# willSapgreen/stereo-vision

Measured on AMD Instinct MI355X. Metric: stereo pairs/sec (ELAS 1242x375, ROBOTICS, D1+D2+LR), higher is better.
Workload: dtype u8

## Files before the change

### include/svh.h

```cpp
#ifndef SVH_H
#define SVH_H

#include <stddef.h>
#include <stdint.h>

#ifdef __cplusplus
extern "C" {
#endif

#define SVH_OK                 0
#define SVH_ERR_FEW_SUPPORT    1
#define SVH_ERR_BAD_ARG       -1
#define SVH_ERR_HIP           -2
#define SVH_ERR_UNSUPPORTED   -3
#define SVH_ERR_NO_DEVICE     -4
#define SVH_ERR_BAD_DIMS      -7

typedef struct svh_elas_params {
    int32_t disp_min;
    int32_t disp_max;
    float   support_threshold;
    int32_t support_texture;
    int32_t candidate_stepsize;
    int32_t incon_window_size;
// ... 96 lines not shown
int32_t svh_elas_stream_push_device(svh_elas_stream* s, const uint8_t* dI1, const uint8_t* dI2,
                                    float* dD1, float* dD2, uint64_t* ticket);
int32_t svh_elas_stream_flush(svh_elas_stream* s);
int32_t svh_elas_stream_pop(svh_elas_stream* s, uint64_t* ticket, int32_t* status, int32_t timeout_ms);
int32_t svh_elas_stream_close(svh_elas_stream* s);
int32_t svh_elas_stream_push_device_n(svh_elas_stream* s, int32_t n, const uint8_t* dI1, const uint8_t* dI2,
                                      size_t in_stride, float* dD1, float* dD2, size_t out_stride,
                                      uint64_t* first_ticket);
int32_t svh_elas_stream_pop_n(svh_elas_stream* s, int32_t n, int32_t* status, int32_t* popped);
int32_t svh_elas_stream_push_n(svh_elas_stream* s, int32_t n, const uint8_t* const* I1, const uint8_t* const* I2,
                               float* const* D1, float* const* D2, uint64_t* first_ticket);

#define SVH_DISP_F32 0
#define SVH_DISP_U16 1
#define SVH_MAPS_BOTH 0
#define SVH_MAPS_LEFT 1
typedef struct { int32_t format; int32_t maps; } svh_elas_output;
int32_t svh_elas_process_out(svh_elas* e, const uint8_t* I1, const uint8_t* I2, void* D1, void* D2,
                             const int32_t* dims, const svh_elas_output* out);
int32_t svh_elas_process_batch_out(svh_elas* e, int32_t n, const uint8_t* const* I1, const uint8_t* const* I2,
                                   void* const* D1, void* const* D2, const int32_t* dims, int32_t* status,
                                   const svh_elas_output* out);
svh_elas_stream* svh_elas_stream_open_out(svh_elas* e, const int32_t* dims, int32_t depth, const svh_elas_output* out);
int32_t svh_elas_stream_push_out(svh_elas_stream* s, const uint8_t* I1, const uint8_t* I2, void* D1, void* D2,
                                 uint64_t* ticket);
int32_t svh_elas_stream_push_out_n(svh_elas_stream* s, int32_t n, const uint8_t* const* I1, const uint8_t* const* I2,
                                   void* const* D1, void* const* D2, uint64_t* first_ticket);
int32_t svh_disparity_pack_u16(const float* D, int32_t d_on_device, int64_t n, uint16_t* out, int32_t out_on_device);
int32_t svh_disparity_unpack_u16(const uint16_t* v, int64_t n, float* out);

int64_t svh_elas_trim(void);

int32_t svh_elas_set_lanes(int32_t lanes);
int32_t svh_elas_set_group(int32_t pairs);

int32_t svh_elas_set_stage(int32_t where);
void svh_elas_stage_stats(int64_t* device_groups, int64_t* handed_back);
void svh_elas_sizing_stats(int64_t* out4);
void svh_elas_get_settings(int32_t out[4]);

enum svh_elas_stage {
    SVH_ELAS_DESC1 = 0,
    SVH_ELAS_DESC2,
    SVH_ELAS_DCAN_RAW,
    SVH_ELAS_SUPPORT,
    SVH_ELAS_TRI1,
    SVH_ELAS_TRI2,
    SVH_ELAS_PLANES1,
    SVH_ELAS_PLANES2,
    SVH_ELAS_GRID1,
    SVH_ELAS_GRID2,
    SVH_ELAS_D1_RAW,
    SVH_ELAS_D2_RAW,
    SVH_ELAS_D1_LR,
    SVH_ELAS_D2_LR,
    SVH_ELAS_D1_SEG,
    SVH_ELAS_D2_SEG,
    SVH_ELAS_D1_GAP,
    SVH_ELAS_D2_GAP,
    SVH_ELAS_STAGE_COUNT
};
int32_t svh_elas_set_taps(svh_elas* e, int32_t enable);
int32_t svh_elas_get_stage(svh_elas* e, int32_t stage, void* buf, size_t cap, size_t* size);

int32_t svh_elas_last_timing(svh_elas* e, const char** names, float* ms, int32_t cap);

// ... 183 lines not shown
```

### stereo-vision_amd/csrc/elas_engine.cpp

```cpp
#include <hip/hip_runtime.h>
#include <stdio.h>
#include <string.h>

#include <atomic>
#include <chrono>
#include <condition_variable>
#include <deque>
#include <functional>
#include <algorithm>
#include <map>
#include <memory>
#include <mutex>
#include <string>
#include <thread>
#include <vector>

#include "hip_guard.h"
#include "svh_internal.h"

namespace svh {

static thread_local int t_device = 0;

#define HIP_TRY(kind, expr) SVH_HIP_TRY(nullptr, kind, expr)
#define LANE_GROW(buf, bytes) SVH_HIP_GROW(nullptr, buf, bytes)

struct KernelStat {
    double total_ms = 0;
    int64_t launches = 0;
};
static std::mutex g_prof_mu;
static std::map<std::string, KernelStat> g_prof;
static std::atomic<int> g_prof_on{0};
static char g_prof_only[64] = "";

struct EventProfiler : Profiler {
    hipStream_t stream = nullptr;
    std::vector<hipEvent_t> ev;
    std::vector<const char*> names;
    size_t used = 0;
    bool skipping = false;
    void begin(const char* kernel) override {
        skipping = g_prof_only[0] && strcmp(kernel, g_prof_only) != 0;
        if (skipping) return;
        if (ev.size() < 2 * (used + 1)) {
            hipEvent_t a, b;
            if (hipEventCreate(&a) != hipSuccess || hipEventCreate(&b) != hipSuccess) return;
            ev.push_back(a);
            ev.push_back(b);
            names.push_back(kernel);
        }
        names[used] = kernel;
        (void)hipEventRecord(ev[2 * used], stream);
    }
    void end() override {
        if (skipping || ev.size() < 2 * (used + 1)) return;
        (void)hipEventRecord(ev[2 * used + 1], stream);
        used++;
    }
    void collect() {
        if (!used) return;
        std::lock_guard<std::mutex> lk(g_prof_mu);
        for (size_t i = 0; i < used; i++) {
            float ms = 0;
            if (hipEventElapsedTime(&ms, ev[2 * i], ev[2 * i + 1]) == hipSuccess) {
                KernelStat& k = g_prof[names[i]];
                k.total_ms += ms;
                k.launches++;
            }
        }
        used = 0;
    }
};

struct LaneBufs {
    HipBuf<uint8_t> img;
    HipBuf<uint8_t> desc;
    HipBuf<int16_t> dcan;
    HipBuf<int32_t> owner;
    HipBuf<uint8_t> prior_dev;
    HipBuf<TriRaster> raster;
    HipBuf<float> planes;
    HipBuf<uint32_t> seed, mask;
    HipBuf<uint16_t> lists;
    HipBuf<float> Draw;
    HipBuf<float> D;
    HipBuf<float> tmp;
    HipBuf<uint16_t> U;
    HipBuf<int32_t> labels, counts;
    HipBuf<int32_t> seg_nroots;
    HipBuf<uint8_t> stage_blob;
    PinnedBuf<int16_t> h_dcan;
    PinnedBuf<uint8_t> h_img, h_prior;
    PinnedBuf<StageCounts> h_counts;
};

struct Lane : LaneBufs {
    EventProfiler prof;
    int device = 0;
    hipStream_t stream = nullptr;
    hipEvent_t wait_ev = nullptr;
    hipStream_t copy_stream = nullptr;
    hipEvent_t match_ev = nullptr, copy_ev = nullptr;
    bool poll_wait = false;
    bool parallel_host = true;
    bool lone_group = true;
    int32_t W = 0, H = 0, disp_max = -1, step = 0, grid_size = 0, sub = -1, gcap = 0;
    Dims d{};
    bool desc_fly = false;
    int64_t owner_hi = 0;
    size_t prior_cap = 0;
    size_t ntri_max = 0;
    std::vector<HostPrior> hp;
    std::vector<int32_t> P;
    StageDev stg{};
    bool stage_ok = false;
    hipEvent_t stage_ev = nullptr;
    bool resident = false;
    bool force_host = false;
    float P_key[5] = {-1, -1, -1, -1, -1};
    static constexpr int kHist = 4;
    int32_t hist_sup[kHist] = {}, hist_tri[kHist] = {};
    int hist_n = 0, hist_at = 0;
    int32_t hist_g = 0;
    svh_elas_params hist_p{};
    PhaseBSize sized{};
    size_t o_P = 0, o_sup = 0, o_tri = 0;

    void release() {
        if (!stream) return;
        (void)hipSetDevice(device);
        static_cast<LaneBufs&>(*this) = LaneBufs();
        stage_ok = false; stg = StageDev{};
        P_key[0] = -1;
        hist_n = 0;
        W = H = 0;
    }

    void destroy() {
        if (!stream) return;
        (void)hipSetDevice(device);
        release();
        for (hipEvent_t* e : {&wait_ev, &match_ev, &copy_ev, &stage_ev})
            if (*e) {
                (void)hipEventDestroy(*e);
                *e = nullptr;
            }
        for (hipEvent_t e : prof.ev) (void)hipEventDestroy(e);
        prof.ev.clear();
        prof.names.clear();
        if (copy_stream) (void)hipStreamDestroy(copy_stream);
        (void)hipStreamDestroy(stream);
        copy_stream = stream = nullptr;
    }

    int ensure(const svh_elas_params& p, int32_t w, int32_t h, int32_t g) {
        if (!stream) {
            HIP_TRY(none, hipSetDevice(device));
            HIP_TRY(none, hipStreamCreateWithFlags(&stream, hipStreamNonBlocking));
        }
        const int32_t st = p.candidate_stepsize + (p.subsampling ? p.candidate_stepsize % 2 : 0);
        if (w == W && h == H && p.disp_max == disp_max && st == step && p.grid_size == grid_size &&
            p.subsampling == sub && g <= gcap)
            return SVH_OK;
        hipStream_t keep = stream;
        release();
        stream = keep;
        d = make_dims(p, w, h);
        const size_t N = (size_t)w * h, DN = (size_t)d.DW * d.DH, G2 = (size_t)2 * g;
        LANE_GROW(img, G2 * N);
        LANE_GROW(desc, G2 * N * 16);
        LANE_GROW(owner, G2 * N * sizeof(int32_t));
        HIP_TRY(copy, hipMemset(owner, 0, G2 * N * sizeof(int32_t)));
        owner_hi = svh::env("SVH_TEST_OWNER_HI") ? atoll(svh::env("SVH_TEST_OWNER_HI")) : 0;
        LANE_GROW(Draw, G2 * DN * sizeof(float));
        LANE_GROW(D, G2 * DN * sizeof(float));
        LANE_GROW(tmp, G2 * DN * sizeof(float));
        LANE_GROW(labels, G2 * DN * sizeof(int32_t));
        LANE_GROW(counts, G2 * DN * sizeof(int32_t));
        LANE_GROW(seg_nroots, G2 * (size_t)((d.DW + 63) / 64) * ((d.DH + 15) / 16) * sizeof(int32_t));
        const size_t nc = (size_t)d.Wc * d.Hc;
        LANE_GROW(dcan, g * nc * sizeof(int16_t));
        LANE_GROW(h_dcan, g * nc * sizeof(int16_t));
        LANE_GROW(h_img, G2 * N);
        const size_t nsup = nc + 6;
        ntri_max = 2 * nsup + 8;
        prior_cap = sizeof(GroupHdr) + (size_t)(p.disp_max + 1) * sizeof(int32_t) + 512 +
                    (size_t)g * (nsup * 3 + 2 * ntri_max * 3) * sizeof(int32_t);
        LANE_GROW(prior_dev, prior_cap);
        LANE_GROW(h_prior, prior_cap);
        LANE_GROW(raster, G2 * ntri_max * sizeof(TriRaster));
        LANE_GROW(planes, G2 * ntri_max * 6 * sizeof(float));
        const size_t gw_bytes = G2 * d.gw * d.gh * d.gwords * sizeof(uint32_t);
        LANE_GROW(seed, gw_bytes + G2 * sizeof(uint32_t));
        LANE_GROW(mask, gw_bytes);
        if (d.gwords <= 8) LANE_GROW(lists, G2 * d.gw * d.gh * 32 * sizeof(uint16_t));
        hp.resize(g);
        o_P = (sizeof(GroupHdr) + 63) & ~(size_t)63;
        o_sup = (o_P + (size_t)(p.disp_max + 1) * sizeof(int32_t) + 63) & ~(size_t)63;
        o_tri = (o_sup + (size_t)g * nsup * 3 * sizeof(int32_t) + 63) & ~(size_t)63;
// ... 30 lines not shown
            stg.rec_cap = (int32_t)rec;
            stage_ok = true;
        }
        HIP_TRY(wait, hipDeviceSynchronize());
        W = w; H = h; disp_max = p.disp_max; step = st; grid_size = p.grid_size; sub = p.subsampling;
        gcap = g;
        return SVH_OK;
    }
};

static std::atomic<int> g_wait_us{40};
static std::atomic<bool> g_hostprof{false};
static hipError_t lane_wait(Lane& L) {
    if (!L.poll_wait || g_wait_us <= 0) return hipStreamSynchronize(L.stream);
    if (!L.wait_ev) {
        hipError_t e = hipEventCreateWithFlags(&L.wait_ev, hipEventDisableTiming);
        if (e != hipSuccess) return e;
    }
    hipError_t e = hipEventRecord(L.wait_ev, L.stream);
    if (e != hipSuccess) return e;
    for (;;) {
        e = hipEventQuery(L.wait_ev);
        if (e != hipErrorNotReady) return e;
        std::this_thread::sleep_for(std::chrono::microseconds(g_wait_us.load(std::memory_order_relaxed)));
    }
}

struct Pool {
    std::mutex mu;
    std::condition_variable cv;
    std::vector<Lane*> lanes;
    std::vector<Lane*> free_list;
    int max_lanes = 4;
};

static std::mutex g_mu;

static std::map<int, Pool*>& g_pools = *new std::map<int, Pool*>();
static std::atomic<int> g_lanes{6};
static std::atomic<int> g_group{32};
static std::atomic<bool> g_group_set{false};
static std::atomic<int> g_stage_mode{-1};
static int stage_mode_from_env();
static void apply_config(const svh_config& c, int explicit_call) {
    if (explicit_call) {
        if (c.elas_workers > 0) svh_elas_set_lanes(c.elas_workers);
        if (c.elas_pairs_per_launch > 0) svh_elas_set_group(c.elas_pairs_per_launch);
        svh_elas_set_stage(c.elas_stage);
        if (c.wait_us >= 0) g_wait_us = c.wait_us;
    }
    if (const char* e = svh::env("SVH_WAIT_US")) g_wait_us = atoi(e);
    if (svh::env("SVH_STAGE")) g_stage_mode.store(stage_mode_from_env());
    g_hostprof = svh::env("SVH_HOST_PROF") != nullptr;
}
namespace { struct ConfigHook { ConfigHook() { svh::on_config(apply_config); } } g_config_hook; }
static int group_for(size_t N) {
    const int g = std::max(1, std::min(g_group.load(), kMaxGroup));
    if (g_group_set.load()) return g;
    size_t a = std::max<size_t>(1, std::min<size_t>(g, (size_t)32 * 1024 * 1024 / std::max<size_t>(N, 1)));
    size_t free_b = 0, total_b = 0;
    if (a > 1 && hipMemGetInfo(&free_b, &total_b) == hipSuccess && free_b > 0) {
        const size_t per_pair = 120 * std::max<size_t>(N, 1), sets = (size_t)2 * std::max(1, g_lanes.load());
        a = std::max<size_t>(1, std::min<size_t>(a, free_b / 2 / (per_pair * sets)));
    } else {
        (void)hipGetLastError();
    }
    return (int)a;
}

static Pool* pool_for(int device) {
    std::lock_guard<std::mutex> lk(g_mu);
    auto it = g_pools.find(device);
    if (it != g_pools.end()) return it->second;
    Pool* p = new Pool();
    g_pools[device] = p;
    return p;
}

static void acquire_lanes(int device, int count, Lane** out) {
    Pool* p = pool_for(device);
    std::unique_lock<std::mutex> lk(p->mu);
    p->max_lanes = 2 * g_lanes.load() + 2;
    for (;;) {
        const int can_make = p->max_lanes - (int)p->lanes.size();
        if ((int)p->free_list.size() + std::max(can_make, 0) >= count) {
            for (int i = 0; i < count; i++) {
                if (!p->free_list.empty()) {
                    out[i] = p->free_list.back();
                    p->free_list.pop_back();
                } else {
                    Lane* l = new Lane();
                    l->device = device;
                    p->lanes.push_back(l);
                    out[i] = l;
                }
            }
            return;
        }
        p->cv.wait(lk);
    }
}

static Lane* acquire_lane(int device) {
    Lane* l = nullptr;
    acquire_lanes(device, 1, &l);
    return l;
}

static void release_lane(Lane* l) {
    Pool* p = pool_for(l->device);
    {
        std::lock_guard<std::mutex> lk(p->mu);
        p->free_list.push_back(l);
    }
    p->cv.notify_all();
}

struct Taps {
    bool enabled = false;
    std::vector<uint8_t> data[SVH_ELAS_STAGE_COUNT];
};

}

struct svh_elas {
    svh_elas_params p;
    int device;
    svh::Taps taps;
// ... 75 lines not shown
};
static HostProfDump g_hp_dump;
#define HP_MARK(slot) do { if (g_hostprof) { uint64_t n_ = cpu_ns(); g_hp_ns[slot] += n_ - hp_t; hp_t = n_; } } while (0)

static int stage_mode_from_env() {
    const char* e = svh::env("SVH_STAGE");
    if (!e || !*e || !strcmp(e, "auto") || !strcmp(e, "-1")) return -1;
    if (!strcmp(e, "host") || !strcmp(e, "0")) return 0;
    if (!strcmp(e, "device") || !strcmp(e, "1")) return 1;
    fprintf(stderr, "svhip: SVH_STAGE=%s is not one of auto|-1, host|0, device|1: using auto\n", e);
    return -1;
}

static std::atomic<int64_t> g_stage_dev_groups{0}, g_stage_redo_groups{0};
static std::atomic<int64_t> g_sized_bound{0}, g_sized_hist{0}, g_short_tri{0}, g_short_sup{0};

static hipError_t event_wait(Lane& L, hipEvent_t ev) {
    if (!L.poll_wait || g_wait_us <= 0) return hipEventSynchronize(ev);
    for (;;) {
        hipError_t e = hipEventQuery(ev);
        if (e != hipErrorNotReady) return e;
        std::this_thread::sleep_for(std::chrono::microseconds(g_wait_us.load(std::memory_order_relaxed)));
    }
}

static int run_group_body(Lane& L, const svh_elas_params& p, const int32_t* dims, const GroupIO& io,
                          int32_t* status, Taps* taps, svh_elas* timing, int mode, int prefer_device);

static int run_group(Lane& L, const svh_elas_params& p, const int32_t* dims, const GroupIO& io,
                     int32_t* status, Taps* taps, svh_elas* timing, int mode = RG_ALL, int prefer_device = 0) {
    const int rc = run_group_body(L, p, dims, io, status, taps, timing, mode, prefer_device);
    if (rc == SVH_ERR_HIP) {
        const std::string keep = svh_last_error();
        if (L.stream) (void)hipStreamSynchronize(L.stream);
        if (L.copy_stream) (void)hipStreamSynchronize(L.copy_stream);
        (void)hipGetLastError();
        L.prof.used = 0;
        L.resident = false;
        L.force_host = false;
        L.P_key[0] = -1;
        fail(rc, keep);
    }
    return rc;
}

static int run_group_body(Lane& L, const svh_elas_params& p, const int32_t* dims, const GroupIO& io,
                          int32_t* status, Taps* taps, svh_elas* timing, int mode, int prefer_device) {
    const int32_t W = dims[0], H = dims[1], g = io.g;
    int rc = check_params(p, W, H);
    if (rc) return rc;
    if (g < 1 || g > kMaxGroup) return fail(SVH_ERR_BAD_ARG, "bad group size");
    HIP_TRY(none, hipSetDevice(L.device));
    rc = L.ensure(p, W, H, g);
    if (rc) return rc;
    if (g > 1) taps = nullptr;
    const Dims& d = L.d;
    const bool u16 = !io.out_device && io.format == SVH_DISP_U16;
    const int nmaps = !io.out_device && io.maps == SVH_MAPS_LEFT ? 1 : 2;
    const size_t DNu = ((size_t)d.DW * d.DH + 7) & ~(size_t)7;
    if (u16) LANE_GROW(L.U, (size_t)L.gcap * 2 * DNu * sizeof(uint16_t));
    hipStream_t s = L.stream;
    L.prof.stream = s;
    const LaunchCtx cx = {s, g_prof_on.load() ? &L.prof : nullptr, L.lone_group};
    const size_t N = (size_t)W * H, DN = (size_t)d.DW * d.DH;
    const size_t nc = (size_t)d.Wc * d.Hc;
    const bool tapping = taps && taps->enabled;
    double t0 = now_ms();
    uint64_t hp_t = g_hostprof ? cpu_ns() : 0;

    GroupHdr* hdr = reinterpret_cast<GroupHdr*>(L.h_prior.p);
    DevMaps out;
    if (io.out_device) {
        out.D[0] = io.dD[0]; out.D[1] = io.dD[1]; out.stride[0] = out.stride[1] = io.out_stride;
    } else {
        out.D[0] = L.D; out.D[1] = L.D + DN; out.stride[0] = out.stride[1] = 2 * DN;
    }
    bool early_d2 = false;
    int32_t plane_radius = 2;

    auto enqueue_phase_b = [&](size_t o_P, size_t o_sup, size_t o_tri, int32_t total_sup, int32_t total_tri,
                               int32_t tri_bound, const PhaseBSize& size) -> int {
        GroupDev G;
        G.hdr = reinterpret_cast<const GroupHdr*>(L.prior_dev.p);
        G.P = reinterpret_cast<const int32_t*>(L.prior_dev + o_P);
        G.support = reinterpret_cast<const int32_t*>(L.prior_dev + o_sup);
        G.tri = reinterpret_cast<const int32_t*>(L.prior_dev + o_tri);
        G.raster = L.raster;
        G.planes = L.planes;
        G.seed = L.seed;
        G.mask = L.mask;
        G.lists = L.lists;
        G.desc = L.desc;
        G.desc_fly = L.desc_fly ? 1 : 0;
        G.owner = L.owner;
        if (L.owner_hi + 1 + tri_bound >= INT32_MAX) {
            HIP_TRY(copy, hipMemsetAsync(L.owner, 0, (size_t)2 * L.gcap * N * sizeof(int32_t), s));
            L.owner_hi = 0;
        }
        G.owner_base = (int32_t)L.owner_hi;
        L.owner_hi += 1 + tri_bound;
        G.Draw = L.Draw;
        G.plane_radius = plane_radius;
        G.prior_absmax = 0;
        for (int32_t dd = 0; dd <= plane_radius && dd < (int32_t)L.P.size(); dd++)
            G.prior_absmax = std::max(G.prior_absmax, (int32_t)std::min<int64_t>(std::llabs((long long)L.P[dd]), INT32_MAX));
        launch_prior(cx, p, d, g, total_sup, total_tri, G, size);
        if (tapping) {
            const int32_t n1 = hdr->tri_end[0], n2 = hdr->tri_end[1] - hdr->tri_end[0];
            rc = tap_dev(L, taps, SVH_ELAS_PLANES1, L.planes.p, (size_t)6 * n1); if (rc) return rc;
            rc = tap_dev(L, taps, SVH_ELAS_PLANES2, L.planes.p + (size_t)6 * n1, (size_t)6 * n2); if (rc) return rc;
            const size_t words = (size_t)d.gw * d.gh * d.gwords;
            std::vector<uint32_t> m(2 * words);
            HIP_TRY(copy, hipMemcpyAsync(m.data(), L.mask, m.size() * sizeof(uint32_t), hipMemcpyDeviceToHost, s));
            HIP_TRY(wait, lane_wait(L));
            for (int k = 0; k < 2; k++) {
                std::vector<int32_t> gr;
                expand_grid(p, d, m.data() + k * words, gr);
                tap_host(taps, SVH_ELAS_GRID1 + k, gr.data(), gr.size());
            }
        }
        launch_owner(cx, p, d, g, total_tri, G, size);
        const bool tiles = !tapping && post_tiles_ok(p);
        const char* match_err = nullptr;
        const bool lr_done = launch_match(cx, p, d, g, G, &out, tapping, &match_err);
        if (match_err) return fail(SVH_ERR_HIP, std::string("launch_match: ") + match_err);
        early_d2 = !io.out_device && lr_done && !tapping && p.postprocess_only_left && !u16 && nmaps == 2;
        if (early_d2) {
            if (!L.copy_stream) {
                HIP_TRY(none, hipStreamCreateWithFlags(&L.copy_stream, hipStreamNonBlocking));
                HIP_TRY(none, hipEventCreateWithFlags(&L.match_ev, hipEventDisableTiming));
                HIP_TRY(none, hipEventCreateWithFlags(&L.copy_ev, hipEventDisableTiming));
            }
            HIP_TRY(none, hipEventRecord(L.match_ev, s));
        }
        if (tapping) {
            rc = tap_dev(L, taps, SVH_ELAS_D1_RAW, L.Draw.p, DN); if (rc) return rc;
            rc = tap_dev(L, taps, SVH_ELAS_D2_RAW, L.Draw.p + DN, DN); if (rc) return rc;
        }
        const PostScratch ps = {L.tmp, L.labels, L.counts, L.seg_nroots};
        const int nside = p.postprocess_only_left ? 1 : 2;
        if (!lr_done) launch_lr(cx, p, d, g, G, out);
        if (tapping) {
            rc = tap_dev(L, taps, SVH_ELAS_D1_LR, out.D[0], DN); if (rc) return rc;
            rc = tap_dev(L, taps, SVH_ELAS_D2_LR, out.D[1], DN); if (rc) return rc;
        }
        launch_segments(cx, p, d, g, nside, G, out, ps, !tiles);
        if (tapping) {
            rc = tap_dev(L, taps, SVH_ELAS_D1_SEG, out.D[0], DN); if (rc) return rc;
            rc = tap_dev(L, taps, SVH_ELAS_D2_SEG, out.D[1], DN); if (rc) return rc;
        }
        if (tiles) {
            launch_gap_mean_tiles(cx, p, d, g, nside, G, out, ps);
        } else {
            launch_gap(cx, p, d, g, nside, G, out, ps);
            if (tapping) {
                rc = tap_dev(L, taps, SVH_ELAS_D1_GAP, out.D[0], DN); if (rc) return rc;
                rc = tap_dev(L, taps, SVH_ELAS_D2_GAP, out.D[1], DN); if (rc) return rc;
            }
            if (p.filter_adaptive_mean) launch_adaptive_mean(cx, p, d, g, nside, G, out, ps);
            if (p.filter_median) launch_median(cx, d, g, nside, G, out, ps);
        }
        if (u16) {
            PackMap pm[2 * kMaxGroup];
            for (int32_t j = 0; j < g; j++)
                for (int k = 0; k < nmaps; k++)
                    pm[j * nmaps + k] = {(int64_t)(((size_t)2 * j + k) * DN), (int64_t)(((size_t)j * nmaps + k) * DNu), (int64_t)DN};
            launch_disp_pack(cx, L.D, L.U, pm, g * nmaps);
        }
        return SVH_OK;
    };

    static const bool strided = !(svh::env("SVH_D2H_STRIDED") && atoi(svh::env("SVH_D2H_STRIDED")) == 0);
    auto copy_map = [&](int k, hipStream_t cs, const int32_t* active) -> int {
        const size_t bytes = DN * (u16 ? sizeof(uint16_t) : sizeof(float));
        const size_t spitch = u16 ? (size_t)nmaps * DNu * sizeof(uint16_t) : 2 * bytes;
        for (int32_t j = 0; j < g;) {
            if (!active[j]) { j++; continue; }
            int32_t e = j + 1;
            while (strided && e < g && active[e] &&
                   reinterpret_cast<const char*>(io.hD[k][e]) == reinterpret_cast<const char*>(io.hD[k][e - 1]) + bytes)
                e++;
            const void* src = u16 ? (const void*)(L.U + ((size_t)j * nmaps + k) * DNu)
                                  : (const void*)(L.D + ((size_t)2 * j + k) * DN);
            if (e - j > 1)
                HIP_TRY(copy, hipMemcpy2DAsync(io.hD[k][j], bytes, src, spitch, bytes, (size_t)(e - j),
                                         hipMemcpyDeviceToHost, cs));
            else
                HIP_TRY(copy, hipMemcpyAsync(io.hD[k][j], src, bytes, hipMemcpyDeviceToHost, cs));
            g_d2h_map_bytes.fetch_add((int64_t)(bytes * (size_t)(e - j)), std::memory_order_relaxed);
            g_d2h_map_copies.fetch_add(1, std::memory_order_relaxed);
            j = e;
        }
        return SVH_OK;
    };
    auto copy_out = [&](const int32_t* active) -> int {
        if (io.out_device) return SVH_OK;
        if (early_d2) {
            HIP_TRY(none, hipStreamWaitEvent(L.copy_stream, L.match_ev, 0));
            rc = copy_map(1, L.copy_stream, active);
            if (rc) return rc;
// ... 100 lines not shown
                        uint8_t* dst = L.h_img + ((size_t)2 * j + k) * N;
                        const uint8_t* src = io.hI[k][j];
                        if (io.pitch == W) memcpy(dst, src, N);
                        else
                            for (int32_t v = 0; v < H; v++) memcpy(dst + (size_t)v * W, src + (size_t)v * io.pitch, W);
                    }
                HIP_TRY(copy, hipMemcpyAsync(L.img, L.h_img, (size_t)2 * g * N, hipMemcpyHostToDevice, s));
            }
            img.I[0] = L.img; img.I[1] = L.img + N;
            img.stride = 2 * N; img.pitch = W;
        }
        {
            std::vector<int32_t> Pt;
            int32_t pr = 2;
            prior_table(p, Pt, &pr);
            int32_t absmax = 0;
            for (int32_t dd = 0; dd <= pr && dd < (int32_t)Pt.size(); dd++)
                absmax = std::max(absmax, (int32_t)std::min<int64_t>(std::llabs((long long)Pt[dd]), INT32_MAX));
            static const int fly_env = svh::env("SVH_DESC_FLY") ? atoi(svh::env("SVH_DESC_FLY")) : 1;
            L.desc_fly = (!tapping || fly_env == 2) && descriptors_on_the_fly(p, d, absmax, pr, L.lists != nullptr);
        }
        if (tapping && L.desc_fly) {
            launch_descriptor(cx, img, g, W, H, p.subsampling, L.desc, false);
            int rc2 = tap_dev(L, taps, SVH_ELAS_DESC1, L.desc.p, N * 16); if (rc2) return rc2;
            rc2 = tap_dev(L, taps, SVH_ELAS_DESC2, L.desc.p + N * 16, N * 16); if (rc2) return rc2;
            HIP_TRY(wait, hipStreamSynchronize(s));
        }
        launch_descriptor(cx, img, g, W, H, p.subsampling, L.desc, L.desc_fly);
        launch_support(cx, p, d, g, L.desc, L.dcan, L.desc_fly);
        const int sm = g_stage_mode.load();
        L.resident = !L.force_host && L.stage_ok &&
                     (sm == 1 || (sm < 0 && prefer_device && stage_device_preferred(p, d, prefer_device > 1)));
        if (L.resident && prefer_device) L.poll_wait = true;
        if (!L.resident || tapping)
            HIP_TRY(copy, hipMemcpyAsync(L.h_dcan, L.dcan, g * nc * sizeof(int16_t), hipMemcpyDeviceToHost, s));
        if (L.resident) {
            prior_table(p, L.P, &plane_radius);
            const float key[5] = {p.beta, p.gamma, p.sigma, p.sradius, (float)p.disp_max};
            if (memcmp(key, L.P_key, sizeof(key)) != 0) {
                memcpy(L.h_prior + L.o_P, L.P.data(), L.P.size() * sizeof(int32_t));
                HIP_TRY(copy, hipMemcpyAsync(L.prior_dev + L.o_P, L.h_prior + L.o_P, L.P.size() * sizeof(int32_t),
                                       hipMemcpyHostToDevice, s));
                HIP_TRY(wait, hipStreamSynchronize(s));
                memcpy(L.P_key, key, sizeof(key));
            }
            if (tapping) {
                HIP_TRY(wait, hipStreamSynchronize(s));
                if (!L.desc_fly) {
                    rc = tap_dev(L, taps, SVH_ELAS_DESC1, L.desc.p, N * 16); if (rc) return rc;
                    rc = tap_dev(L, taps, SVH_ELAS_DESC2, L.desc.p + N * 16, N * 16); if (rc) return rc;
                }
                tap_host(taps, SVH_ELAS_DCAN_RAW, L.h_dcan.p, nc);
            }
            const bool blits = svh::env("SVH_STAGE_BLITS") && atoi(svh::env("SVH_STAGE_BLITS")) != 0;
            launch_stage_device(cx, p, d, g, L.stg, reinterpret_cast<GroupHdr*>(L.prior_dev.p),
                                reinterpret_cast<int32_t*>(L.prior_dev + L.o_sup),
                                reinterpret_cast<int32_t*>(L.prior_dev + L.o_tri),
                                blits ? nullptr : L.seed.p, seed_words_with_flags(d, g),
                                blits ? nullptr : L.h_counts.p);
            if (!L.stage_ev) HIP_TRY(none, hipEventCreateWithFlags(&L.stage_ev, hipEventDisableTiming));
            if (blits) HIP_TRY(copy, hipMemcpyAsync(L.h_counts, L.stg.counts, sizeof(StageCounts), hipMemcpyDeviceToHost, s));
            HIP_TRY(none, hipEventRecord(L.stage_ev, s));
            if (tapping) {
                HIP_TRY(copy, hipMemcpyAsync(hdr, L.prior_dev, sizeof(GroupHdr), hipMemcpyDeviceToHost, s));
                HIP_TRY(wait, hipStreamSynchronize(s));
                if (hdr->active[0]) {
                    rc = tap_dev(L, taps, SVH_ELAS_SUPPORT, reinterpret_cast<int32_t*>(L.prior_dev + L.o_sup),
                                 (size_t)3 * hdr->total_sup); if (rc) return rc;
                    rc = tap_dev(L, taps, SVH_ELAS_TRI1, reinterpret_cast<int32_t*>(L.prior_dev + L.o_tri),
                                 (size_t)3 * hdr->tri_end[0]); if (rc) return rc;
                    rc = tap_dev(L, taps, SVH_ELAS_TRI2,
                                 reinterpret_cast<int32_t*>(L.prior_dev + L.o_tri) + (size_t)3 * hdr->tri_end[0],
                                 (size_t)3 * (hdr->tri_end[1] - hdr->tri_end[0])); if (rc) return rc;
                }
            }
            L.sized = PhaseBSize{};
            if (!tapping || hdr->active[0]) {
                const int32_t tri_bound = 2 * g * 2 * L.stg.sup_cap;
                int32_t hint_sup = 0, hint_tri = 0;
                const bool use_hist = !(svh::env("SVH_PHASEB_HISTORY") && atoi(svh::env("SVH_PHASEB_HISTORY")) == 0);
                if (use_hist && L.hist_n && L.hist_g == g && memcmp(&L.hist_p, &p, sizeof(p)) == 0)
                    for (int k = 0; k < L.hist_n; k++) {
                        hint_sup = std::max(hint_sup, L.hist_sup[k]);
                        hint_tri = std::max(hint_tri, L.hist_tri[k]);
                    }
                L.sized = phase_b_size(d, g, -1, -1, hint_sup, hint_tri);
                L.sized.seed_cleared = !blits;
                rc = enqueue_phase_b(L.o_P, L.o_sup, L.o_tri, -1, -1, tri_bound, L.sized);
                if (rc) return rc;
            }
        }
        HP_MARK(HP_ENQ_A);
    }
    if (!(mode & RG_HOST_B)) return SVH_OK;
    double t1 = t0, t2 = t0;
    if (L.resident) {
        if (!io.out_device) {
            HIP_TRY(wait, event_wait(L, L.stage_ev));
            HP_MARK(HP_WAIT);
            int32_t active[kMaxGroup];
            for (int32_t j = 0; j < g; j++) active[j] = active_of(j);
            rc = copy_out(active);
            if (rc) return rc;
        }
        if (g_hostprof) g_hp_pairs += g;
        HP_MARK(HP_ENQ_B);
        t1 = t2 = now_ms();
    } else {
    const bool warm = L.parallel_host && g == 1;
    if (warm) helpers_warm(3, 1500);
    struct WarmOff {
        bool on;
        ~WarmOff() { if (on) helpers_warm(0, 0); }
    } warm_off{warm};
    HIP_TRY(wait, lane_wait(L));
    HIP_TRY(launch, hipGetLastError());
    L.prof.collect();
    HP_MARK(HP_WAIT);
    if (g_hostprof) g_hp_pairs += g;
    t1 = now_ms();
    if (tapping) {
        if (!L.desc_fly) {
// ... 888 lines not shown

void svh_test_d2h_map_bytes(int64_t out[2], int32_t reset) {
    if (out) {
        out[0] = svh::g_d2h_map_bytes.load();
        out[1] = svh::g_d2h_map_copies.load();
    }
    if (reset) {
        svh::g_d2h_map_bytes.store(0);
        svh::g_d2h_map_copies.store(0);
    }
}

void svh_elas_sizing_stats(int64_t* out4) {
    if (!out4) return;
    out4[0] = svh::g_sized_bound.load();
    out4[1] = svh::g_sized_hist.load();
    out4[2] = svh::g_short_tri.load();
    out4[3] = svh::g_short_sup.load();
}

void svh_elas_stage_stats(int64_t* device_groups, int64_t* handed_back) {
    if (device_groups) *device_groups = g_stage_dev_groups.load();
    if (handed_back) *handed_back = g_stage_redo_groups.load();
}

void svh_elas_get_settings(int32_t out[4]) {
    if (!out) return;
    out[0] = g_lanes.load();
    out[1] = g_group_set.load() ? g_group.load() : 0;
    out[2] = g_stage_mode.load();
    out[3] = g_wait_us;
}

int32_t svh_elas_set_group(int32_t pairs) {
    if (pairs < 1) pairs = 1;
    if (pairs > kMaxGroup) pairs = kMaxGroup;
    g_group.store(pairs);
    g_group_set.store(true);
    return pairs;
}

}
```

### stereo-vision_amd/svhip/__init__.py

```python
import ctypes as C
import os

import numpy as np

_HERE = os.path.dirname(os.path.abspath(__file__))
LIB_PATH = os.environ.get("SVH_LIB") or os.path.join(os.path.dirname(_HERE), "libsvhip.so")

OK, ERR_FEW_SUPPORT, ERR_BAD_ARG, ERR_HIP, ERR_UNSUPPORTED, ERR_NO_DEVICE = 0, 1, -1, -2, -3, -4
ERR_BAD_DIMS = -7
ROBOTICS, MIDDLEBURY = 0, 1


class ElasParams(C.Structure):
    _fields_ = [
        ("disp_min", C.c_int32), ("disp_max", C.c_int32),
        ("support_threshold", C.c_float), ("support_texture", C.c_int32),
        ("candidate_stepsize", C.c_int32), ("incon_window_size", C.c_int32),
        ("incon_threshold", C.c_int32), ("incon_min_support", C.c_int32),
        ("add_corners", C.c_int32), ("grid_size", C.c_int32),
        ("beta", C.c_float), ("gamma", C.c_float), ("sigma", C.c_float), ("sradius", C.c_float),
        ("match_texture", C.c_int32), ("lr_threshold", C.c_int32),
        ("speckle_sim_threshold", C.c_float), ("speckle_size", C.c_int32),
        ("ipol_gap_width", C.c_int32), ("filter_median", C.c_int32),
        ("filter_adaptive_mean", C.c_int32), ("postprocess_only_left", C.c_int32),
# ... 355 lines not shown

    def set_taps(self, enable=True):
        lib().svh_elas_set_taps(self._h, 1 if enable else 0)

    def stage(self, stage, dtype):
        n = C.c_size_t(0)
        lib().svh_elas_get_stage(self._h, stage, None, 0, C.byref(n))
        buf = np.empty(n.value, np.uint8)
        if n.value:
            rc = lib().svh_elas_get_stage(self._h, stage, buf.ctypes.data, n.value, C.byref(n))
            if rc < 0:
                raise SvhError(rc, last_error())
        return buf.view(dtype)

    def last_timing(self):
        names = (C.c_char_p * 16)()
        ms = (C.c_float * 16)()
        n = lib().svh_elas_last_timing(self._h, names, ms, 16)
        return [(names[i].decode(), ms[i]) for i in range(n)]


def set_lanes(n):
    return lib().svh_elas_set_lanes(n)


def set_group(n):
    return lib().svh_elas_set_group(n)


def set_stage(where):
    return lib().svh_elas_set_stage(where)


def trim():
    lib().svh_elas_trim.restype = C.c_int64
    return lib().svh_elas_trim()


def stage_stats():
    a, b = C.c_int64(0), C.c_int64(0)
    lib().svh_elas_stage_stats(C.byref(a), C.byref(b))
    return a.value, b.value


def device_count():
    return lib().svh_device_count()


def pack_u16(D):
    D = np.ascontiguousarray(D, np.float32)
    out = np.empty(D.shape, np.uint16)
    rc = lib().svh_disparity_pack_u16(D.ctypes.data, 0, D.size, out.ctypes.data, 0)
    if rc < 0:
        raise SvhError(rc, last_error())
    return out


def unpack_u16(v):
    v = np.ascontiguousarray(v, np.uint16)
    out = np.empty(v.shape, np.float32)
    rc = lib().svh_disparity_unpack_u16(v.ctypes.data, v.size, out.ctypes.data)
    if rc < 0:
        raise SvhError(rc, last_error())
    return out


# ... 454 lines not shown
```

Before: 35630.

## Split ELAS phases across priority-classed HIP streams per lane

Adds a queue plan that gives each lane up to three HIP streams with different priorities and routes phase A, the device staging phase and phase B (match, LR, postprocess) onto separate streams joined by events. Lanes of alternating parity can get low-priority streams, so concurrent lanes interleave better on the GPU's hardware queues. The auto plan picks by GPU_MAX_HW_QUEUES and the worker count, and falls back to a single stream when queues are plentiful or the budget is exceeded. This adds event synchronisation overhead, and the extra streams risk contending for the limited hardware queues.

```diff
diff --git a/include/svh.h b/include/svh.h
--- a/include/svh.h
+++ b/include/svh.h
@@ -152,6 +152,8 @@
 int64_t svh_elas_trim(void);
 
 int32_t svh_elas_set_lanes(int32_t lanes);
+int32_t svh_elas_set_queue_plan(int32_t plan);
+int32_t svh_elas_get_queue_plan(int32_t* plan, int32_t* streams_per_lane, int32_t* classes);
 int32_t svh_elas_set_group(int32_t pairs);
 
 int32_t svh_elas_set_stage(int32_t where);
diff --git a/stereo-vision_amd/csrc/elas_engine.cpp b/stereo-vision_amd/csrc/elas_engine.cpp
--- a/stereo-vision_amd/csrc/elas_engine.cpp
+++ b/stereo-vision_amd/csrc/elas_engine.cpp
@@ -16,6 +16,7 @@
 #include <vector>
 
 #include "hip_guard.h"
+#include "queue_plan.h"
 #include "svh_internal.h"
 
 namespace svh {
@@ -72,6 +73,20 @@
         used = 0;
     }
 };
+
+struct PhaseProfiler : Profiler {
+    EventProfiler* to;
+    hipStream_t stream;
+    PhaseProfiler(EventProfiler* t, hipStream_t s) : to(t), stream(s) {}
+    void begin(const char* kernel) override {
+        to->stream = stream;
+        to->begin(kernel);
+    }
+    void end() override { to->end(); }
+};
+
+static int queue_cap();
+static int worker_count();
 
 struct LaneBufs {
     HipBuf<uint8_t> img;
@@ -98,7 +113,15 @@
 struct Lane : LaneBufs {
     EventProfiler prof;
     int device = 0;
-    hipStream_t stream = nullptr;
+    hipStream_t stream = nullptr, stage_stream = nullptr, post_stream = nullptr;
+    hipStream_t cls_stream[QC_COUNT] = {nullptr, nullptr, nullptr};
+    int plan_req = QP_AUTO;
+    int parity = 0;
+    bool qp_known = false;
+    QueuePlan qp{};
+    int prio_least = 0, prio_greatest = 0;
+    bool split = false;
+    hipEvent_t a_ev = nullptr, b_ev = nullptr;
     hipEvent_t wait_ev = nullptr;
     hipStream_t copy_stream = nullptr;
     hipEvent_t match_ev = nullptr, copy_ev = nullptr;
@@ -138,10 +161,10 @@
     }
 
     void destroy() {
-        if (!stream) return;
+        if (!cls_stream[QC_NORMAL] && !cls_stream[QC_HIGH] && !cls_stream[QC_LOW]) return;
         (void)hipSetDevice(device);
         release();
-        for (hipEvent_t* e : {&wait_ev, &match_ev, &copy_ev, &stage_ev})
+        for (hipEvent_t* e : {&wait_ev, &match_ev, &copy_ev, &stage_ev, &a_ev, &b_ev})
             if (*e) {
                 (void)hipEventDestroy(*e);
                 *e = nullptr;
@@ -150,22 +173,48 @@
         prof.ev.clear();
         prof.names.clear();
         if (copy_stream) (void)hipStreamDestroy(copy_stream);
-        (void)hipStreamDestroy(stream);
-        copy_stream = stream = nullptr;
+        for (hipStream_t& cs : cls_stream)
+            if (cs) {
+                (void)hipStreamDestroy(cs);
+                cs = nullptr;
+            }
+        copy_stream = stream = stage_stream = post_stream = nullptr;
+    }
+
+    int bind_streams() {
+        if (!qp_known) {
+            HIP_TRY(none, hipSetDevice(device));
+            if (hipDeviceGetStreamPriorityRange(&prio_least, &prio_greatest) != hipSuccess) {
+                (void)hipGetLastError();
+                prio_least = prio_greatest = 0;
+            }
+            qp = make_queue_plan(prio_least, prio_greatest, queue_cap(), worker_count(), plan_req);
+            qp_known = true;
+        }
+        const QueueLane& ql = qp.lane[parity & 1];
+        for (int k = 0; k < ql.nstreams; k++) {
+            hipStream_t& cs = cls_stream[ql.cls[k]];
+            if (cs) continue;
+            HIP_TRY(none, hipSetDevice(device));
+            if (qp.plan == QP_ONE)
+                HIP_TRY(none, hipStreamCreateWithFlags(&cs, hipStreamNonBlocking));
+            else
+                HIP_TRY(none, hipStreamCreateWithPriority(&cs, hipStreamNonBlocking,
+                                                          queue_priority_of(ql.cls[k], prio_least, prio_greatest)));
+        }
+        stream = cls_stream[ql.cls[ql.phase_stream[QPH_A]]];
+        stage_stream = cls_stream[ql.cls[ql.phase_stream[QPH_S]]];
+        post_stream = cls_stream[ql.cls[ql.phase_stream[QPH_B]]];
+        return SVH_OK;
     }
 
     int ensure(const svh_elas_params& p, int32_t w, int32_t h, int32_t g) {
-        if (!stream) {
-            HIP_TRY(none, hipSetDevice(device));
-            HIP_TRY(none, hipStreamCreateWithFlags(&stream, hipStreamNonBlocking));
-        }
+        if (int rc = bind_streams()) return rc;
         const int32_t st = p.candidate_stepsize + (p.subsampling ? p.candidate_stepsize % 2 : 0);
         if (w == W && h == H && p.disp_max == disp_max && st == step && p.grid_size == grid_size &&
             p.subsampling == sub && g <= gcap)
             return SVH_OK;
-        hipStream_t keep = stream;
         release();
-        stream = keep;
         d = make_dims(p, w, h);
         const size_t N = (size_t)w * h, DN = (size_t)d.DW * d.DH, G2 = (size_t)2 * g;
         LANE_GROW(img, G2 * N);
@@ -262,6 +311,7 @@
     std::vector<Lane*> lanes;
     std::vector<Lane*> free_list;
     int max_lanes = 4;
+    int queue_plan = -2;
 };
 
 static std::mutex g_mu;
@@ -272,6 +322,10 @@
 static std::atomic<bool> g_group_set{false};
 static std::atomic<int> g_stage_mode{-1};
 static int stage_mode_from_env();
+static std::atomic<int> g_queue_plan{QP_AUTO};
+static std::atomic<int> g_queue_cap{kQueueCapDefault};
+static int queue_cap() { return g_queue_cap.load(); }
+static int worker_count() { return g_lanes.load(); }
 static void apply_config(const svh_config& c, int explicit_call) {
     if (explicit_call) {
         if (c.elas_workers > 0) svh_elas_set_lanes(c.elas_workers);
@@ -282,6 +336,11 @@
     if (const char* e = svh::env("SVH_WAIT_US")) g_wait_us = atoi(e);
     if (svh::env("SVH_STAGE")) g_stage_mode.store(stage_mode_from_env());
     g_hostprof = svh::env("SVH_HOST_PROF") != nullptr;
+    g_queue_cap = queue_cap_from_text(getenv("GPU_MAX_HW_QUEUES"));
+    if (const char* e = svh::env("SVH_QUEUE_PLAN")) {
+        const int v = atoi(e);
+        g_queue_plan = v >= 0 && v <= QP_LAST ? v : QP_AUTO;
+    }
 }
 namespace { struct ConfigHook { ConfigHook() { svh::on_config(apply_config); } } g_config_hook; }
 static int group_for(size_t N) {
@@ -321,9 +380,11 @@
                 } else {
                     Lane* l = new Lane();
                     l->device = device;
+                    l->plan_req = p->queue_plan != -2 ? p->queue_plan : g_queue_plan.load();
                     p->lanes.push_back(l);
                     out[i] = l;
                 }
+                out[i]->parity = i;
             }
             return;
         }
@@ -465,7 +526,9 @@
     const int rc = run_group_body(L, p, dims, io, status, taps, timing, mode, prefer_device);
     if (rc == SVH_ERR_HIP) {
         const std::string keep = svh_last_error();
-        if (L.stream) (void)hipStreamSynchronize(L.stream);
+        for (hipStream_t cs : L.cls_stream)
+            if (cs) (void)hipStreamSynchronize(cs);
+        L.split = false;
         if (L.copy_stream) (void)hipStreamSynchronize(L.copy_stream);
         (void)hipGetLastError();
         L.prof.used = 0;
@@ -492,9 +555,11 @@
     const int nmaps = !io.out_device && io.maps == SVH_MAPS_LEFT ? 1 : 2;
     const size_t DNu = ((size_t)d.DW * d.DH + 7) & ~(size_t)7;
     if (u16) LANE_GROW(L.U, (size_t)L.gcap * 2 * DNu * sizeof(uint16_t));
-    hipStream_t s = L.stream;
-    L.prof.stream = s;
-    const LaunchCtx cx = {s, g_prof_on.load() ? &L.prof : nullptr, L.lone_group};
+    hipStream_t s = L.stream, ss = s, sb = L.split ? L.post_stream : s;
+    const bool prof_on = g_prof_on.load() != 0;
+    PhaseProfiler prof_a(&L.prof, s), prof_s(&L.prof, s), prof_b(&L.prof, sb);
+    const LaunchCtx cx = {s, prof_on ? &prof_a : nullptr, L.lone_group};
+    LaunchCtx cx_s = cx, cx_b = {sb, prof_on ? &prof_b : nullptr, L.lone_group};
     const size_t N = (size_t)W * H, DN = (size_t)d.DW * d.DH;
     const size_t nc = (size_t)d.Wc * d.Hc;
     const bool tapping = taps && taps->enabled;
@@ -527,7 +592,7 @@
         G.desc_fly = L.desc_fly ? 1 : 0;
         G.owner = L.owner;
         if (L.owner_hi + 1 + tri_bound >= INT32_MAX) {
-            HIP_TRY(copy, hipMemsetAsync(L.owner, 0, (size_t)2 * L.gcap * N * sizeof(int32_t), s));
+            HIP_TRY(copy, hipMemsetAsync(L.owner, 0, (size_t)2 * L.gcap * N * sizeof(int32_t), sb));
             L.owner_hi = 0;
         }
         G.owner_base = (int32_t)L.owner_hi;
@@ -537,7 +602,7 @@
         G.prior_absmax = 0;
         for (int32_t dd = 0; dd <= plane_radius && dd < (int32_t)L.P.size(); dd++)
             G.prior_absmax = std::max(G.prior_absmax, (int32_t)std::min<int64_t>(std::llabs((long long)L.P[dd]), INT32_MAX));
-        launch_prior(cx, p, d, g, total_sup, total_tri, G, size);
+        launch_prior(cx_b, p, d, g, total_sup, total_tri, G, size);
         if (tapping) {
             const int32_t n1 = hdr->tri_end[0], n2 = hdr->tri_end[1] - hdr->tri_end[0];
             rc = tap_dev(L, taps, SVH_ELAS_PLANES1, L.planes.p, (size_t)6 * n1); if (rc) return rc;
@@ -552,10 +617,10 @@
                 tap_host(taps, SVH_ELAS_GRID1 + k, gr.data(), gr.size());
             }
         }
-        launch_owner(cx, p, d, g, total_tri, G, size);
+        launch_owner(cx_b, p, d, g, total_tri, G, size);
         const bool tiles = !tapping && post_tiles_ok(p);
         const char* match_err = nullptr;
-        const bool lr_done = launch_match(cx, p, d, g, G, &out, tapping, &match_err);
+        const bool lr_done = launch_match(cx_b, p, d, g, G, &out, tapping, &match_err);
         if (match_err) return fail(SVH_ERR_HIP, std::string("launch_match: ") + match_err);
         early_d2 = !io.out_device && lr_done && !tapping && p.postprocess_only_left && !u16 && nmaps == 2;
         if (early_d2) {
@@ -564,7 +629,7 @@
                 HIP_TRY(none, hipEventCreateWithFlags(&L.match_ev, hipEventDisableTiming));
                 HIP_TRY(none, hipEventCreateWithFlags(&L.copy_ev, hipEventDisableTiming));
             }
-            HIP_TRY(none, hipEventRecord(L.match_ev, s));
+            HIP_TRY(none, hipEventRecord(L.match_ev, sb));
         }
         if (tapping) {
             rc = tap_dev(L, taps, SVH_ELAS_D1_RAW, L.Draw.p, DN); if (rc) return rc;
@@ -572,33 +637,33 @@
         }
         const PostScratch ps = {L.tmp, L.labels, L.counts, L.seg_nroots};
         const int nside = p.postprocess_only_left ? 1 : 2;
-        if (!lr_done) launch_lr(cx, p, d, g, G, out);
+        if (!lr_done) launch_lr(cx_b, p, d, g, G, out);
         if (tapping) {
             rc = tap_dev(L, taps, SVH_ELAS_D1_LR, out.D[0], DN); if (rc) return rc;
             rc = tap_dev(L, taps, SVH_ELAS_D2_LR, out.D[1], DN); if (rc) return rc;
         }
-        launch_segments(cx, p, d, g, nside, G, out, ps, !tiles);
+        launch_segments(cx_b, p, d, g, nside, G, out, ps, !tiles);
         if (tapping) {
             rc = tap_dev(L, taps, SVH_ELAS_D1_SEG, out.D[0], DN); if (rc) return rc;
             rc = tap_dev(L, taps, SVH_ELAS_D2_SEG, out.D[1], DN); if (rc) return rc;
         }
         if (tiles) {
-            launch_gap_mean_tiles(cx, p, d, g, nside, G, out, ps);
+            launch_gap_mean_tiles(cx_b, p, d, g, nside, G, out, ps);
         } else {
-            launch_gap(cx, p, d, g, nside, G, out, ps);
+            launch_gap(cx_b, p, d, g, nside, G, out, ps);
             if (tapping) {
                 rc = tap_dev(L, taps, SVH_ELAS_D1_GAP, out.D[0], DN); if (rc) return rc;
                 rc = tap_dev(L, taps, SVH_ELAS_D2_GAP, out.D[1], DN); if (rc) return rc;
             }
-            if (p.filter_adaptive_mean) launch_adaptive_mean(cx, p, d, g, nside, G, out, ps);
-            if (p.filter_median) launch_median(cx, d, g, nside, G, out, ps);
+            if (p.filter_adaptive_mean) launch_adaptive_mean(cx_b, p, d, g, nside, G, out, ps);
+            if (p.filter_median) launch_median(cx_b, d, g, nside, G, out, ps);
         }
         if (u16) {
             PackMap pm[2 * kMaxGroup];
             for (int32_t j = 0; j < g; j++)
                 for (int k = 0; k < nmaps; k++)
                     pm[j * nmaps + k] = {(int64_t)(((size_t)2 * j + k) * DN), (int64_t)(((size_t)j * nmaps + k) * DNu), (int64_t)DN};
-            launch_disp_pack(cx, L.D, L.U, pm, g * nmaps);
+            launch_disp_pack(cx_b, L.D, L.U, pm, g * nmaps);
         }
         return SVH_OK;
     };
@@ -765,6 +830,13 @@
         L.resident = !L.force_host && L.stage_ok &&
                      (sm == 1 || (sm < 0 && prefer_device && stage_device_preferred(p, d, prefer_device > 1)));
         if (L.resident && prefer_device) L.poll_wait = true;
+        L.split = L.resident && !L.lone_group && !tapping && (L.stage_stream != s || L.post_stream != s);
+        ss = L.split ? L.stage_stream : s;
+        sb = L.split ? L.post_stream : s;
+        prof_s.stream = ss;
+        prof_b.stream = sb;
+        cx_s = LaunchCtx{ss, prof_on ? &prof_s : nullptr, L.lone_group};
+        cx_b = LaunchCtx{sb, prof_on ? &prof_b : nullptr, L.lone_group};
         if (!L.resident || tapping)
             HIP_TRY(copy, hipMemcpyAsync(L.h_dcan, L.dcan, g * nc * sizeof(int16_t), hipMemcpyDeviceToHost, s));
         if (L.resident) {
@@ -786,14 +858,20 @@
                 tap_host(taps, SVH_ELAS_DCAN_RAW, L.h_dcan.p, nc);
             }
             const bool blits = svh::env("SVH_STAGE_BLITS") && atoi(svh::env("SVH_STAGE_BLITS")) != 0;
-            launch_stage_device(cx, p, d, g, L.stg, reinterpret_cast<GroupHdr*>(L.prior_dev.p),
+            if (ss != s) {
+                if (!L.a_ev) HIP_TRY(none, hipEventCreateWithFlags(&L.a_ev, hipEventDisableTiming));
+                HIP_TRY(none, hipEventRecord(L.a_ev, s));
+                HIP_TRY(none, hipStreamWaitEvent(ss, L.a_ev, 0));
+            }
+            launch_stage_device(cx_s, p, d, g, L.stg, reinterpret_cast<GroupHdr*>(L.prior_dev.p),
                                 reinterpret_cast<int32_t*>(L.prior_dev + L.o_sup),
                                 reinterpret_cast<int32_t*>(L.prior_dev + L.o_tri),
                                 blits ? nullptr : L.seed.p, seed_words_with_flags(d, g),
                                 blits ? nullptr : L.h_counts.p);
             if (!L.stage_ev) HIP_TRY(none, hipEventCreateWithFlags(&L.stage_ev, hipEventDisableTiming));
-            if (blits) HIP_TRY(copy, hipMemcpyAsync(L.h_counts, L.stg.counts, sizeof(StageCounts), hipMemcpyDeviceToHost, s));
-            HIP_TRY(none, hipEventRecord(L.stage_ev, s));
+            if (blits) HIP_TRY(copy, hipMemcpyAsync(L.h_counts, L.stg.counts, sizeof(StageCounts), hipMemcpyDeviceToHost, ss));
+            HIP_TRY(none, hipEventRecord(L.stage_ev, ss));
+            if (sb != ss) HIP_TRY(none, hipStreamWaitEvent(sb, L.stage_ev, 0));
             if (tapping) {
                 HIP_TRY(copy, hipMemcpyAsync(hdr, L.prior_dev, sizeof(GroupHdr), hipMemcpyDeviceToHost, s));
                 HIP_TRY(wait, hipStreamSynchronize(s));
@@ -821,6 +899,11 @@
                 L.sized.seed_cleared = !blits;
                 rc = enqueue_phase_b(L.o_P, L.o_sup, L.o_tri, -1, -1, tri_bound, L.sized);
                 if (rc) return rc;
+            }
+            if (sb != s) {
+                if (!L.b_ev) HIP_TRY(none, hipEventCreateWithFlags(&L.b_ev, hipEventDisableTiming));
+                HIP_TRY(none, hipEventRecord(L.b_ev, sb));
+                HIP_TRY(none, hipStreamWaitEvent(s, L.b_ev, 0));
             }
         }
         HP_MARK(HP_ENQ_A);
@@ -1775,6 +1858,36 @@
     out[3] = g_wait_us;
 }
 
+int32_t svh_elas_set_queue_plan(int32_t plan) {
+    svh::ensure_init();
+    if (plan < 0 || plan > QP_LAST) plan = QP_AUTO;
+    Pool* p = pool_for(t_device);
+    std::lock_guard<std::mutex> lk(p->mu);
+    p->queue_plan = plan;
+    return plan;
+}
+
+int32_t svh_elas_get_queue_plan(int32_t* plan, int32_t* streams_per_lane, int32_t* classes) {
+    svh::ensure_init();
+    Pool* p = pool_for(t_device);
+    int req;
+    {
+        std::lock_guard<std::mutex> lk(p->mu);
+        req = p->queue_plan != -2 ? p->queue_plan : g_queue_plan.load();
+    }
+    int least = 0, greatest = 0, n = 0;
+    if (hipGetDeviceCount(&n) != hipSuccess || n <= t_device || hipSetDevice(t_device) != hipSuccess ||
+        hipDeviceGetStreamPriorityRange(&least, &greatest) != hipSuccess) {
+        (void)hipGetLastError();
+        least = greatest = 0;
+    }
+    const QueuePlan q = make_queue_plan(least, greatest, queue_cap(), worker_count(), req);
+    if (plan) *plan = q.plan;
+    if (streams_per_lane) *streams_per_lane = q.streams_per_lane;
+    if (classes) *classes = q.classes;
+    return SVH_OK;
+}
+
 int32_t svh_elas_set_group(int32_t pairs) {
     if (pairs < 1) pairs = 1;
     if (pairs > kMaxGroup) pairs = kMaxGroup;
diff --git a/stereo-vision_amd/csrc/queue_plan.h b/stereo-vision_amd/csrc/queue_plan.h
--- /dev/null
+++ b/stereo-vision_amd/csrc/queue_plan.h
@@ -0,0 +1,97 @@
+#ifndef SVH_QUEUE_PLAN_H
+#define SVH_QUEUE_PLAN_H
+
+#include <stdlib.h>
+
+namespace svh {
+
+enum { QC_NORMAL = 0, QC_HIGH = 1, QC_LOW = 2, QC_COUNT = 3 };
+enum { QPH_A = 0, QPH_S = 1, QPH_B = 2, QPH_COUNT = 3 };
+enum { QP_AUTO = -1, QP_ONE = 0, QP_STAGE_HIGH = 1, QP_SECOND_LOW = 2, QP_BY_PHASE = 3, QP_PARITY = 4, QP_LAST = 4 };
+
+constexpr int kQueueCapDefault = 4;
+constexpr int kQueueBudget = 12;
+constexpr int kQueuePlanWhenShort = QP_PARITY;
+
+struct QueueLane {
+    int nstreams;
+    int cls[QC_COUNT];
+    int phase_stream[QPH_COUNT];
+};
+struct QueuePlan {
+    int plan;
+    QueueLane lane[2];
+    int streams_per_lane;
+    int classes;
+    int queues;
+};
+
+inline int queue_cap_from_text(const char* text) {
+    if (!text || !*text) return kQueueCapDefault;
+    const long v = strtol(text, nullptr, 10);
+    if (v <= 0) return kQueueCapDefault;
+    return v > 1024 ? 1024 : (int)v;
+}
+
+inline int queue_priority_normal(int least, int greatest) { return 0 < greatest ? greatest : (0 > least ? least : 0); }
+inline int queue_fold_class(int cls, int least, int greatest) {
+    const int normal = queue_priority_normal(least, greatest);
+    if (cls == QC_HIGH && greatest < normal) return QC_HIGH;
+    if (cls == QC_LOW && least > normal) return QC_LOW;
+    return QC_NORMAL;
+}
+inline int queue_priority_of(int cls, int least, int greatest) {
+    return cls == QC_HIGH ? greatest : cls == QC_LOW ? least : queue_priority_normal(least, greatest);
+}
+
+inline void queue_plan_wanted(int plan, int parity, int out[QPH_COUNT]) {
+    out[QPH_A] = out[QPH_S] = out[QPH_B] = QC_NORMAL;
+    if (plan == QP_STAGE_HIGH || plan == QP_SECOND_LOW) out[QPH_S] = QC_HIGH;
+    if ((plan == QP_SECOND_LOW || plan == QP_PARITY) && parity == 1) out[QPH_A] = out[QPH_B] = QC_LOW;
+    if (plan == QP_PARITY && parity == 1) out[QPH_S] = QC_LOW;
+    if (plan == QP_BY_PHASE) {
+        out[QPH_S] = QC_HIGH;
+        out[QPH_B] = QC_LOW;
+    }
+}
+
+inline QueuePlan queue_plan_layout(int least, int greatest, int cap, int workers, int plan) {
+    QueuePlan q{};
+    q.plan = plan;
+    int per_class[QC_COUNT] = {0, 0, 0};
+    for (int parity = 0; parity < 2; parity++) {
+        QueueLane& L = q.lane[parity];
+        int want[QPH_COUNT];
+        queue_plan_wanted(plan, parity, want);
+        for (int ph = 0; ph < QPH_COUNT; ph++) {
+            const int c = queue_fold_class(want[ph], least, greatest);
+            int k = 0;
+            while (k < L.nstreams && L.cls[k] != c) k++;
+            if (k == L.nstreams) L.cls[L.nstreams++] = c;
+            L.phase_stream[ph] = k;
+        }
+        for (int k = 0; k < L.nstreams; k++) per_class[L.cls[k]] += workers;
+        if (L.nstreams > q.streams_per_lane) q.streams_per_lane = L.nstreams;
+    }
+    for (int c = 0; c < QC_COUNT; c++)
+        if (per_class[c]) {
+            q.classes++;
+            q.queues += per_class[c] < cap ? per_class[c] : cap;
+        }
+    return q;
+}
+
+inline QueuePlan make_queue_plan(int least, int greatest, int cap, int workers, int requested) {
+    if (least < greatest) { const int t = least; least = greatest; greatest = t; }
+    if (cap < 1) cap = 1;
+    if (workers < 1) workers = 1;
+    int plan = requested;
+    if (plan < 0 || plan > QP_LAST) plan = cap < 2 * workers ? kQueuePlanWhenShort : QP_ONE;
+    QueuePlan q = queue_plan_layout(least, greatest, cap, workers, plan);
+    if (plan != QP_ONE && q.queues > kQueueBudget) q = queue_plan_layout(least, greatest, cap, workers, QP_ONE);
+    if (q.streams_per_lane == 1 && q.classes == 1) q.plan = QP_ONE;
+    return q;
+}
+
+}
+#endif
diff --git a/stereo-vision_amd/svhip/__init__.py b/stereo-vision_amd/svhip/__init__.py
--- a/stereo-vision_amd/svhip/__init__.py
+++ b/stereo-vision_amd/svhip/__init__.py
@@ -411,6 +411,16 @@
     return lib().svh_elas_set_stage(where)
 
 
+def set_queue_plan(plan):
+    return lib().svh_elas_set_queue_plan(int(plan))
+
+
+def queue_plan():
+    p, s, c = C.c_int32(-9), C.c_int32(-9), C.c_int32(-9)
+    lib().svh_elas_get_queue_plan(C.byref(p), C.byref(s), C.byref(c))
+    return dict(plan=p.value, streams_per_lane=s.value, classes=c.value)
+
+
 def trim():
     lib().svh_elas_trim.restype = C.c_int64
     return lib().svh_elas_trim()
```

Result: faster. 36480 (median of 6 runs) (+2.4%).
